# hrnr/map-merge

Hardware: AMD Instinct MI355X
Metric: map-pairs/sec (normals+FPFH+SAC-IA+ICP, end to end incl. per-map features) (higher is better)
Workload: dtype f32; 1 GPU; 16 maps x 500000 raw pts, FPFH + SAC_IA + ICP refine, 120 pairs; parallelism=one mm3d_estimate_maps_transforms call, 16 streams inside the library, points_after_filter_mean=406681, keypoints_mean=15692

## Files before the change

include/mm3d.h:

```cpp
#ifndef MM3D_H_
#define MM3D_H_

#include <stddef.h>
#include <stdint.h>

#ifdef __cplusplus
extern "C" {
#endif

typedef enum {
  MM3D_OK = 0,
  MM3D_EINVAL = -1,
  MM3D_EDEVICE = -2,
  MM3D_ENOMEM = -3,
  MM3D_EUNSUPPORTED = -4,
  MM3D_ECAPACITY = -5
} mm3d_status;

typedef enum { MM3D_DESC_PFH = 0, MM3D_DESC_PFHRGB, MM3D_DESC_FPFH, MM3D_DESC_RSD, MM3D_DESC_SHOT, MM3D_DESC_SC3D } mm3d_descriptor;
typedef enum { MM3D_KP_SIFT = 0, MM3D_KP_HARRIS } mm3d_keypoint;
typedef enum { MM3D_EST_MATCHING = 0, MM3D_EST_SAC_IA } mm3d_estimation_method;
typedef enum { MM3D_ICP_POINT_TO_POINT = 0, MM3D_ICP_POINT_TO_PLANE = 1 } mm3d_icp_method;

const char *mm3d_descriptor_name(int d);
int mm3d_descriptor_from_string(const char *s);
const char *mm3d_descriptor_field_name(int d);
int mm3d_descriptor_dim(int d);
const char *mm3d_keypoint_name(int k);
int mm3d_keypoint_from_string(const char *s);
const char *mm3d_estimation_method_name(int m);
int mm3d_estimation_method_from_string(const char *s);

typedef struct {
  double resolution;
  double descriptor_radius;
  int outliers_min_neighbours;
  double normal_radius;
  int keypoint_type;
  double keypoint_threshold;
  int descriptor_type;
  int estimation_method;
  int refine_transform;
  double inlier_threshold;
  double max_correspondence_distance;
  int max_iterations;
  uint64_t matching_k;
  double transform_epsilon;
  double confidence_threshold;
  double output_resolution;
} mm3d_params;
void mm3d_params_default(mm3d_params *p);
int mm3d_params_from_command_line(int argc, const char *const *argv, mm3d_params *p);
size_t mm3d_params_to_string(const mm3d_params *p, char *buf, size_t cap);

typedef struct { int32_t index_query, index_match; float distance; } mm3d_corr;

typedef struct mm3d_ctx mm3d_ctx;
typedef struct mm3d_cloud mm3d_cloud;
typedef struct mm3d_normals mm3d_normals;
typedef struct mm3d_desc mm3d_desc;

int mm3d_create(int device, mm3d_ctx **out);
int mm3d_create_devices(const int *devices, int n_devices, mm3d_ctx **out);
int mm3d_device_count(const mm3d_ctx *ctx);
int mm3d_device_at(const mm3d_ctx *ctx, int i);
int mm3d_devices_use_rccl(const mm3d_ctx *ctx);
void mm3d_destroy(mm3d_ctx *ctx);
const char *mm3d_last_error(const mm3d_ctx *ctx);
int mm3d_last_icp_iterations(const mm3d_ctx *ctx);
int mm3d_last_icp_converged(const mm3d_ctx *ctx);
void mm3d_set_debug(mm3d_ctx *ctx, int on);
long long mm3d_debug_knn_fallback_rows(mm3d_ctx *ctx);
long long mm3d_debug_knn_rows(mm3d_ctx *ctx);
void mm3d_debug_waits(mm3d_ctx *ctx, long long out[2]);
int mm3d_debug_float_chain(mm3d_ctx *ctx, const float *incr, const unsigned *hits, int n, float *out);
int mm3d_debug_libm(mm3d_ctx *ctx, int fn, const float *x, const float *y, int n, float *out);
int mm3d_debug_pair_bins(mm3d_ctx *ctx, const float *p1, const float *n1, const float *p2, const float *n2, int n, int *out);
void mm3d_debug_spfh_replay(const float *incr, const unsigned *hits, int n, float *out);
int mm3d_debug_sacia_queries_per_thread(int k);
int mm3d_debug_wave_primitives(mm3d_ctx *ctx, int op, const void *in, int n, void *out_new, void *out_old);
int mm3d_debug_sift_cert_octave(mm3d_ctx *ctx, const mm3d_cloud *points, double min_scale, int octave, float *val, float *bound,
                                size_t capacity, size_t *n_out);
void mm3d_debug_sift_cert_stats(long long out[8], int reset);
void mm3d_debug_sift_cert_min(int n);
int mm3d_debug_sift_dog_marked(mm3d_ctx *ctx, const mm3d_cloud *points, double min_scale, int octave, const int *ids, size_t n_ids,
                               int small_capacity, float *out);
float mm3d_debug_cloud_voxel_leaf(const mm3d_cloud *cloud);
void mm3d_debug_sacia_stats(long long out[4], int reset, int collect);
int mm3d_debug_desc_knn(mm3d_ctx *ctx, const float *a, size_t na, const float *b, size_t nb, int dim, int k, int *idx, float *d2);
typedef struct mm3d_nn_search_info {
  float max_d2;
  float rmax;
  float cell;
  float origin[3];
  int dims[3];
  int max_ring;
  int n_items;
} mm3d_nn_search_info;
int mm3d_debug_nn_search(mm3d_ctx *ctx, const mm3d_cloud *source, const mm3d_cloud *target, const float T[16], double range,
                         int convention, int split, int *idx, float *d2, mm3d_nn_search_info *info);
void mm3d_srand(mm3d_ctx *ctx, unsigned seed);
int mm3d_set_streams(mm3d_ctx *ctx, int n_streams);
int mm3d_get_streams(const mm3d_ctx *ctx);
int mm3d_last_run_stage_seconds(const mm3d_ctx *ctx, double *features_s, double *total_s);
int mm3d_last_run_device_seconds(const mm3d_ctx *ctx, double *exchange_s, double *pairs_s, double *gather_s);
size_t mm3d_last_run_map_sizes(const mm3d_ctx *ctx, size_t *points, size_t *keypoints, size_t capacity);
int mm3d_set_map_cache(mm3d_ctx *ctx, int max_maps);
int mm3d_get_map_cache(const mm3d_ctx *ctx);
void mm3d_map_cache_clear(mm3d_ctx *ctx);
int mm3d_map_cache_stats(const mm3d_ctx *ctx, long long out[6], int reset);
int mm3d_set_icp_method(mm3d_ctx *ctx, int method);
int mm3d_get_icp_method(const mm3d_ctx *ctx);
typedef enum { MM3D_ALIGN_SAC_IA = 0, MM3D_ALIGN_PREREJECTIVE = 1 } mm3d_align_method;
typedef struct mm3d_alignment_options {
  int method;
  int samples;
  int k;
  double similarity;
  double inlier_fraction;
} mm3d_alignment_options;
typedef struct mm3d_alignment_stats {
  long long draws;
  long long survivors;
  long long hypotheses_scored;
  long long winner_h;
  int winner_inliers;
  int converged;
} mm3d_alignment_stats;
void mm3d_alignment_options_default(mm3d_alignment_options *o);
int mm3d_set_alignment(mm3d_ctx *ctx, const mm3d_alignment_options *options);
int mm3d_get_alignment(const mm3d_ctx *ctx, mm3d_alignment_options *options);
int mm3d_last_alignment_stats(const mm3d_ctx *ctx, mm3d_alignment_stats *stats);
typedef enum { MM3D_KEYPOINTS_REFERENCE = 0, MM3D_KEYPOINTS_UNIFORM = 1 } mm3d_keypoint_source;
typedef struct mm3d_keypoint_options {
  int source;
  double leaf;
} mm3d_keypoint_options;
void mm3d_keypoint_options_default(mm3d_keypoint_options *o);
int mm3d_set_keypoints(mm3d_ctx *ctx, const mm3d_keypoint_options *options);
int mm3d_get_keypoints(const mm3d_ctx *ctx, mm3d_keypoint_options *options);
typedef enum { MM3D_OUTLIERS_RADIUS = 0, MM3D_OUTLIERS_STATISTICAL = 1 } mm3d_outlier_method;
typedef struct mm3d_outlier_options {
  int method;
  int mean_k;
  double stddev_mult;
} mm3d_outlier_options;
void mm3d_outlier_options_default(mm3d_outlier_options *o);
int mm3d_set_outlier_filter(mm3d_ctx *ctx, const mm3d_outlier_options *options);
int mm3d_get_outlier_filter(const mm3d_ctx *ctx, mm3d_outlier_options *options);
typedef struct mm3d_outlier_stats {
  long long points, valid, kept;
  int k;
  double mean, stddev, threshold;
} mm3d_outlier_stats;
int mm3d_last_outlier_stats(const mm3d_ctx *ctx, mm3d_outlier_stats *stats);
typedef enum { MM3D_CLUSTERS_OFF = 0, MM3D_CLUSTERS_MIN_SIZE = 1, MM3D_CLUSTERS_LARGEST = 2 } mm3d_cluster_method;
typedef struct mm3d_cluster_options {
  int method;
  int min_size;
  double tolerance;
} mm3d_cluster_options;
void mm3d_cluster_options_default(mm3d_cluster_options *o);
int mm3d_set_cluster_filter(mm3d_ctx *ctx, const mm3d_cluster_options *options);
int mm3d_get_cluster_filter(const mm3d_ctx *ctx, mm3d_cluster_options *options);
typedef struct mm3d_cluster_stats {
  long long points, valid, kept;
  long long clusters, kept_clusters;
  long long largest;
} mm3d_cluster_stats;
int mm3d_last_cluster_stats(const mm3d_ctx *ctx, mm3d_cluster_stats *stats);
typedef enum { MM3D_SMOOTH_OFF = 0, MM3D_SMOOTH_MLS = 1 } mm3d_smooth_method;
// ... 343 lines not shown
```

map-merge_amd/__init__.py:

```python
from __future__ import annotations

import ctypes as C
import enum
import os
import subprocess

import numpy as np

_HERE = os.path.dirname(os.path.abspath(__file__))
LIB_PATH = os.environ.get("MM3D_LIB") or os.path.join(_HERE, "libmm3d.so")

POINT = np.dtype([("x", "<f4"), ("y", "<f4"), ("z", "<f4"), ("rgba", "<u4")])
NORMAL = np.dtype([("nx", "<f4"), ("ny", "<f4"), ("nz", "<f4"), ("curvature", "<f4")])
CORR = np.dtype([("index_query", "<i4"), ("index_match", "<i4"), ("distance", "<f4")])
PAIR = np.dtype([("source_idx", "<u8"), ("target_idx", "<u8"), ("transform", "<f4", (16,)),
                 ("confidence", "<f8"), ("icp_iterations", "<i4"), ("n_correspondences", "<i4"),
                 ("n_inliers", "<i4"), ("icp_correspondences", "<i4")])


class Mm3dError(RuntimeError):
    def __init__(self, status, msg):
        super().__init__(f"mm3d status {status}: {msg}")
        self.status = status

# ... 1058 lines not shown

    def estimateTransformCorrelative(self, source_points, source_normals, target_points, target_normals, options=None, **kw):
        o = options if options is not None else CoarseOptions(**kw)
        T = np.zeros(16, dtype=np.float32)
        st = CoarseStats()
        self._ck(lib().mm3d_estimate_transform_correlative(
            self._h, source_points._h, source_normals._h, target_points._h, target_normals._h, C.byref(o),
            T.ctypes.data_as(C.c_void_p), C.byref(st)))
        return _Tout(T), st.as_dict()

    def correlativeSignature(self, points, normals, options=None, cap=1 << 20, **kw):
        o = options if options is not None else CoarseOptions(**kw)
        c = max(int(cap), 1)
        st = np.zeros((c, 3), dtype=np.int32)
        gr = np.zeros((c, 3), dtype=np.int32)
        gh = np.zeros(c, dtype=np.float32)
        co = np.zeros((c, 2), dtype=np.int32)
        n = (C.c_size_t * 3)()
        self._ck(lib().mm3d_debug_correlative_signature(
            self._h, points._h, normals._h, C.byref(o), st.ctypes.data_as(C.c_void_p), gr.ctypes.data_as(C.c_void_p),
            gh.ctypes.data_as(C.c_void_p), co.ctypes.data_as(C.c_void_p), C.c_size_t(c), n))
        if max(n) > c:
            raise RuntimeError("correlativeSignature: more cells than cap")
        return dict(structure=st[:n[0]].copy(), ground=gr[:n[1]].copy(), ground_height=gh[:n[1]].copy(), coarse=co[:n[2]].copy())

    def correlativeVotes(self, source_points, source_normals, target_points, target_normals, q, options=None, **kw):
        o = options if options is not None else CoarseOptions(**kw)
        frame = (C.c_int * 5)()
        n = C.c_size_t()
        K, W, GW = int(o.candidates), 2 * int(o.cell_factor) + 1, 2 * int(o.yaw_factor) + 1
        cands = np.zeros((K, 4), dtype=np.int32)
        scores = np.zeros((K, GW, W, W), dtype=np.int32)
        args = (self._h, source_points._h, source_normals._h, target_points._h, target_normals._h, C.byref(o), int(q), frame)
        self._ck(lib().mm3d_debug_correlative_votes(*args, None, C.c_size_t(0), cands.ctypes.data_as(C.c_void_p),
                                                    scores.ctypes.data_as(C.c_void_p), C.c_size_t(K), C.byref(n)))
        U, V = int(frame[3]), int(frame[4])
        acc = np.zeros((U, V), dtype=np.int32)
        if U * V:
            self._ck(lib().mm3d_debug_correlative_votes(*args, acc.ctypes.data_as(C.c_void_p), C.c_size_t(U * V),
                                                        cands.ctypes.data_as(C.c_void_p), scores.ctypes.data_as(C.c_void_p),
                                                        C.c_size_t(K), C.byref(n)))
        m = int(n.value)
        return dict(frame=tuple(int(x) for x in frame), acc=acc, cands=cands[:m].copy(), scores=scores[:m].copy())

    def transformOverlap(self, source_points, target_points, transform, options=None, **kw) -> dict:
        o = options if options is not None else ConfidenceOptions(**kw)
        T = _T(transform)
        st = OverlapStats()
        self._ck(lib().mm3d_transform_overlap(self._h, source_points._h, target_points._h, T.ctypes.data_as(C.c_void_p), C.byref(o),
                                              C.byref(st)))
        return st.as_dict()

    def debugOverlapTable(self, points, options=None, **kw) -> dict:
        o = options if options is not None else ConfidenceOptions(**kw)
        box = (C.c_int * 12)()
        self._ck(lib().mm3d_debug_overlap_table(self._h, points._h, C.byref(o), box, None, C.c_size_t(0), None, C.c_size_t(0)))
        b = [int(x) for x in box]
        words = np.zeros(tuple(b[3:6]), dtype=np.uint64)
        view = np.zeros(tuple(b[9:12]), dtype=np.uint8)
        if words.size:
            self._ck(lib().mm3d_debug_overlap_table(self._h, points._h, C.byref(o), box, words.ctypes.data_as(C.c_void_p),
                                                    C.c_size_t(words.size), view.ctypes.data_as(C.c_void_p), C.c_size_t(view.size)))
        return dict(brick0=tuple(b[0:3]), bricks=tuple(b[3:6]), view0=tuple(b[6:9]), views=tuple(b[9:12]), words=words, view=view)

    def estimateTransform(self, source_points, source_keypoints, source_descriptors, target_points,
                          target_keypoints, target_descriptors, method, refine, inlier_threshold,
                          max_correspondence_distance, max_iterations, matching_k, transform_epsilon):
        T = np.zeros(16, dtype=np.float32)
        self._ck(lib().mm3d_estimate_transform(
            self._h, source_points._h, source_keypoints._h, source_descriptors._h, target_points._h,
            target_keypoints._h, target_descriptors._h, int(method), int(bool(refine)), C.c_double(inlier_threshold),
            C.c_double(max_correspondence_distance), int(max_iterations), C.c_size_t(matching_k),
            C.c_double(transform_epsilon), T.ctypes.data_as(C.c_void_p)))
        return _Tout(T)

    def debugWavePrimitives(self, op, values):
        dt = {0: np.float64, 1: np.float32, 5: np.float32, 6: np.float32, 8: np.uint64}.get(int(op), np.int32)
        v = np.ascontiguousarray(values, dtype=dt)
        new, old = np.empty_like(v), np.empty_like(v)
        self._ck(lib().mm3d_debug_wave_primitives(self._h, int(op), v.ctypes.data_as(C.c_void_p), len(v),
                                                  new.ctypes.data_as(C.c_void_p), old.ctypes.data_as(C.c_void_p)))
        return new, old

    def debugNnSearch(self, source_points, target_points, transform, range, convention, split):
        n = len(source_points)
        idx = np.zeros(max(n, 1), dtype=np.int32)
        d2 = np.zeros(max(n, 1), dtype=np.float32)
        t = _T(transform)
        info = NnSearchInfo()
        self._ck(lib().mm3d_debug_nn_search(self._h, source_points._h, target_points._h, t.ctypes.data_as(C.c_void_p),
                                            C.c_double(range), int(convention), int(split), idx.ctypes.data_as(C.c_void_p),
                                            d2.ctypes.data_as(C.c_void_p), C.byref(info)))
        return idx[:n], d2[:n], info.as_dict()

    def debugColorGradients(self, points, normals, options=None, **kw):
        o = options if options is not None else IcpColorOptions(**kw)
        n = len(points)
        out = np.zeros((max(n, 1), 4), dtype=np.float32)
        self._ck(lib().mm3d_debug_color_gradients(self._h, points._h, normals._h, C.byref(o), out.ctypes.data_as(C.c_void_p)))
        return out[:n]

    def debugIcpRejection(self, source_points, target_points, transform, max_correspondence_distance, options=None, split=1, **kw):
        o = options if options is not None else IcpRejectionOptions(**kw)
        n = len(source_points)
        idx = np.zeros(max(n, 1), dtype=np.int32)
        d2 = np.zeros(max(n, 1), dtype=np.float32)
        kept = np.zeros(max(n, 1), dtype=np.uint8)
        t = _T(transform)
        st = IcpRejectionStats()
        self._ck(lib().mm3d_debug_icp_rejection(self._h, source_points._h, target_points._h, t.ctypes.data_as(C.c_void_p),
                                                C.c_double(max_correspondence_distance), C.byref(o), int(split),
                                                idx.ctypes.data_as(C.c_void_p), d2.ctypes.data_as(C.c_void_p),
                                                kept.ctypes.data_as(C.c_void_p), C.byref(st)))
        return idx[:n], d2[:n], kept[:n].astype(bool), st.as_dict()

    def transformScore(self, source_points, target_points, transform, max_distance) -> float:
        t = _T(transform)
        s = C.c_double()
        self._ck(lib().mm3d_transform_score(self._h, source_points._h, target_points._h, t.ctypes.data_as(C.c_void_p),
                                            C.c_double(max_distance), C.byref(s)))
        return s.value

    def estimateMapsTransforms(self, clouds, params: MapMergingParams, return_pairs: bool = False):
        n = len(clouds)
        keep = []
        views = (_View * max(n, 1))()
        for i, c in enumerate(clouds):
            if isinstance(c, tuple):
                views[i] = _View(C.c_void_p(c[0]), c[1], c[2] if len(c) > 2 else 16, c[3] if len(c) > 3 else 12)
            else:
                a = np.ascontiguousarray(c, dtype=POINT)
                keep.append(a)
                views[i] = _View(a.ctypes.data_as(C.c_void_p), len(a), 16, 12)
        out = np.zeros((max(n, 1), 16), dtype=np.float32)
        pairs = np.zeros(max(n * (n - 1) // 2, 1), dtype=PAIR)
        n_out, n_pairs = C.c_size_t(), C.c_size_t()
        self._ck(lib().mm3d_estimate_maps_transforms(self._h, views, C.c_size_t(n), C.byref(params),
                                                     out.ctypes.data_as(C.c_void_p), C.byref(n_out),
                                                     pairs.ctypes.data_as(C.c_void_p), C.byref(n_pairs)))
        res = [_Tout(out[i]) for i in range(n_out.value)]
        return (res, pairs[:n_pairs.value].copy()) if return_pairs else res

    def composeMaps(self, clouds, transforms, resolution: float):
        n = len(clouds)
        if n == 0:
            return None
        if n != len(transforms):
            raise RuntimeError("composeMaps: clouds and transforms size must be the same.")
        arr = (C.c_void_p * n)(*[c._h for c in clouds])
        tr = np.ascontiguousarray(np.stack([_T(t) for t in transforms]))
        h = C.c_void_p()
        self._ck(lib().mm3d_compose_maps(self._h, arr, C.c_size_t(n), tr.ctypes.data_as(C.c_void_p), C.c_size_t(n),
                                         C.c_double(resolution), C.byref(h)))
        return Cloud(self, h)

    def mapFeatures(self, raw: "Cloud", params: MapMergingParams) -> "Map":
        h = C.c_void_p()
        self._ck(lib().mm3d_map_features(self._h, raw._h, C.byref(params), C.byref(h)))
        return Map(self, h)

    def mapFromParts(self, points: "Cloud", keypoints: "Cloud", desc: "Descriptors") -> "Map":
        h = C.c_void_p()
        self._ck(lib().mm3d_map_from_parts(self._h, points._h, keypoints._h, desc._h, C.byref(h)))
        for o in (points, keypoints, desc):
            o._owned = False
        return Map(self, h)
# ... 190 lines not shown
```

map-merge_amd/csrc/registration.hip:

```cpp
#include <atomic>
#include <cfloat>
#include <cstdlib>

#include "device_util.hpp"
#include "linalg_shared.hpp"

namespace mm3d {

__global__ void __launch_bounds__(256)
k_ransac_count(const float4 *__restrict__ skp, const float4 *__restrict__ tkp, const int *__restrict__ is,
               const int *__restrict__ it, int n_corr, const float *__restrict__ T_all, int H, float thr_le,
               int *__restrict__ counts)
{
  const int h = blockIdx.x * (blockDim.x >> 6) + (threadIdx.x >> 6);
  if (h >= H) return;
  const int lane = threadIdx.x & 63;
  float T[16];
#pragma unroll
  for (int k = 0; k < 16; ++k) T[k] = T_all[(size_t)h * 16 + k];
  int cnt = 0;
  for (int i = lane; i < n_corr; i += kWave) {
    const float4 s = skp[is[i]], t = tkp[it[i]];
    const float3 p = xform(T, s.x, s.y, s.z);
    const float dx = p.x - t.x, dy = p.y - t.y, dz = p.z - t.z;
    const float d = __fadd_rn(__fadd_rn(__fmul_rn(dx, dx), __fmul_rn(dy, dy)), __fmul_rn(dz, dz));
    cnt += (d <= thr_le) ? 1 : 0;
  }
  cnt = wave_sum(cnt);
  if (lane == 0) counts[h] = cnt;
}

void ransac_count(Context *c, const float4 *src_kp, const float4 *tgt_kp, const int *idx_src, const int *idx_tgt,
                  int n_corr, const float *T_all, int H, double thr2, int *counts)
{
  float thr_le = (float)thr2;
  if ((double)thr_le >= thr2) thr_le = std::nextafterf(thr_le, -INFINITY);
  MM3D_LAUNCH(c, "ransac_count", (double)H * n_corr * 8.0, k_ransac_count, dim3(div_up(H, 4)), dim3(256), 0, src_kp, tgt_kp,
              idx_src, idx_tgt, n_corr, T_all, H, thr_le, counts);
}

struct SacJob {
  const float4 *skp, *tkp;
  const int *samp, *corr_ref, *nn;
  float *T_all;
  const float4 *skp_q;
  int ns;
  GridView g;
  float *err;
  float *T_best;
  double *S;
  int *n_part;
  int *chain_list;
  unsigned char *cls;
  struct SacCtl *ctl;
};
struct SacCtl { int n_cand, decided, winner, n_chain; };

__global__ void k_sacia_models(const SacJob *__restrict__ jobs, int H)
{
  const SacJob &J = jobs[blockIdx.y];
  const float4 *__restrict__ skp = J.skp, *__restrict__ tkp = J.tkp;
  const int *__restrict__ samp = J.samp, *__restrict__ corr_ref = J.corr_ref, *__restrict__ nn = J.nn;
  float *__restrict__ T_all = J.T_all;
  const int h = blockIdx.x * blockDim.x + threadIdx.x;
  if (h >= H) return;
  float s[9], d[9], T[16];
#pragma unroll
  for (int i = 0; i < 3; ++i) {
    const float4 p = skp[samp[h * 3 + i]], q = tkp[nn[corr_ref[h * 3 + i]]];
    s[i * 3] = p.x; s[i * 3 + 1] = p.y; s[i * 3 + 2] = p.z;
    d[i * 3] = q.x; d[i * 3 + 1] = q.y; d[i * 3 + 2] = q.z;
  }
  umeyama_f32_shared(s, d, 3, T);
#pragma unroll
  for (int i = 0; i < 16; ++i) T_all[(size_t)h * 16 + i] = T[i];
}

#ifndef MM3D_SAC_SUB
#define MM3D_SAC_SUB 1
#endif
constexpr int kSacSub = MM3D_SAC_SUB;
struct SacQuery { float3 p; int b, e; float slack; bool inside; };
__device__ __forceinline__ SacQuery sacia_locate(const GridView &g, const float *Tl, const float4 s)
{
  SacQuery q;
  q.p = xform(Tl, s.x, s.y, s.z);
  const int cx = cell_floor(q.p.x, g.minx, g.inv), cy = cell_floor(q.p.y, g.miny, g.inv), cz = cell_floor(q.p.z, g.minz, g.inv);
  q.inside = cx >= 0 && cx < g.dx && cy >= 0 && cy < g.dy && cz >= 0 && cz < g.dz;
  const size_t c = q.inside ? ((size_t)cz * g.dy + cy) * g.dx + cx : 0;
  q.b = g.nb_start[c];
  q.e = g.nb_start[c + 1];
  const float ox = q.p.x - (g.minx + ((float)cx + 0.5f) * g.cell), oy = q.p.y - (g.miny + ((float)cy + 0.5f) * g.cell);
  const float oz = q.p.z - (g.minz + ((float)cz + 0.5f) * g.cell);
  q.slack = sqrtf(ox * ox + oy * oy + oz * oz) + 1e-3f * g.cell;
  return q;
}
__device__ __forceinline__ float sacia_scan(const GridView &g, const SacQuery &q, float thresh, float radius)
{
  const float3 p = q.p;
  float best = INFINITY;
  if (q.inside) {
    const int e = q.e;
    float want = thresh;
    for (int j = q.b; j < e; j += 4) {
      const int last = e - 1;
      const float4 q0 = g.nb_pts[j];
      const float4 q1 = g.nb_pts[min(j + 1, last)];
      const float4 q2 = g.nb_pts[min(j + 2, last)];
      const float4 q3 = g.nb_pts[min(j + 3, last)];
      const float d0 = dist2(p.x, p.y, p.z, q0.x, q0.y, q0.z), d1 = dist2(p.x, p.y, p.z, q1.x, q1.y, q1.z);
      const float d2 = dist2(p.x, p.y, p.z, q2.x, q2.y, q2.z), d3 = dist2(p.x, p.y, p.z, q3.x, q3.y, q3.z);
      best = fminf(best, fminf(fminf(d0, d1), fminf(d2, d3)));
      want = fminf(want, best);
      const float lb = q3.w - q.slack;
      if (lb > 0.0f && lb * lb > want) break;
    }
  } else {
    for_each_candidate(g, p.x, p.y, p.z, radius, [&](const float4 &t) {
      best = fminf(best, dist2(p.x, p.y, p.z, t.x, t.y, t.z));
      return true;
    });
  }
  return (best <= thresh) ? best / thresh : 1.0f;
}
__device__ __forceinline__ float sacia_term(const GridView &g, const float *Tl, const float4 s, float thresh, float radius)
{
  return sacia_scan(g, sacia_locate(g, Tl, s), thresh, radius);
}

template <int K>
__global__ void __launch_bounds__(256)
k_sacia_err(const SacJob *__restrict__ jobs, int h_first, float thresh, float radius)
{
  const SacJob &J = jobs[blockIdx.z];
  const int ns = J.ns;
  const int i0 = (int)blockIdx.x * (256 * K);
  if (i0 >= ns) return;
  const int h = h_first + (int)blockIdx.y;
  const float *T = J.T_all + (size_t)h * 16;
  float Tl[16];
#pragma unroll
  for (int k = 0; k < 16; ++k) Tl[k] = T[k];
  float4 s[K];
#pragma unroll
  for (int k = 0; k < K; ++k) {
    const int i = i0 + k * 256 + (int)threadIdx.x;
    s[k] = J.skp_q[i < ns ? i : i0];
  }
  SacQuery q[K];
#pragma unroll
  for (int k = 0; k < K; ++k) q[k] = sacia_locate(J.g, Tl, s[k]);
  double sum = 0.0;
  int part = 0;
#pragma unroll
  for (int k = 0; k < K; ++k) {
    const bool valid = i0 + k * 256 + (int)threadIdx.x < ns;
    const float e_term = valid ? sacia_scan(J.g, q[k], thresh, radius) : 0.0f;
    sum += (double)e_term;
    part += (valid && e_term != 1.0f) ? 1 : 0;
  }
  __shared__ double s_sum[4];
  __shared__ int s_part[4];
  const double ws = wave_sum(sum);
  part = wave_sum(part);
  if ((threadIdx.x & 63) == 0) { s_sum[threadIdx.x >> 6] = ws; s_part[threadIdx.x >> 6] = part; }
  __syncthreads();
  if (threadIdx.x == 0) {
    atomicAdd(&J.S[h], (s_sum[0] + s_sum[1]) + (s_sum[2] + s_sum[3]));
    const int pt = s_part[0] + s_part[1] + s_part[2] + s_part[3];
    if (pt) atomicAdd(&J.n_part[h], pt);
  }
}
#ifndef MM3D_SAC_K
#define MM3D_SAC_K 4
#endif
constexpr int kSacK = MM3D_SAC_K;
constexpr long long kSacMinTiles = 256 * 8;
static std::atomic<int> g_sacia_k{[] { const char *e = getenv("MM3D_SAC_K"); return e ? atoi(e) : 0; }()};
static int sacia_queries_per_thread(long long ns_total, int hn)
{
  const int knob = g_sacia_k.load();
  if (knob == 1 || knob == 2 || knob == 4 || knob == 8) return knob;
  int k = kSacK;
  while (k > 1 && div_up(ns_total, 256 * k) * hn < kSacMinTiles) k >>= 1;
  return k;
}

__global__ void __launch_bounds__(256) k_sacia_select(const SacJob *__restrict__ jobs, int H)
{
  const SacJob &J = jobs[blockIdx.x];
  const double *__restrict__ S = J.S;
  const int *__restrict__ n_part = J.n_part;
  const double n = (double)J.ns;
  const double d = n * 5.9604644775390625e-8 * 1.001 + 1e-12;
  __shared__ double s_min[4];
  __shared__ int s_cnt[4], s_chain[4], s_first[4];
  const int lane = threadIdx.x & 63, wave = threadIdx.x >> 6;
  double up = INFINITY;
  for (int h = threadIdx.x; h < H; h += blockDim.x) {
    const double hi = n_part[h] == 0 ? n : S[h] * (1.0 + d);
    up = hi < up ? hi : up;
  }
#pragma unroll
  for (int o = 32; o > 0; o >>= 1) { const double t = __shfl_xor(up, o, kWave); up = t < up ? t : up; }
  if (lane == 0) s_min[wave] = up;
  __syncthreads();
  up = fmin(fmin(s_min[0], s_min[1]), fmin(s_min[2], s_min[3]));
  int cnt = 0, chain = 0, first = 0x7fffffff;
  for (int h = threadIdx.x; h < H; h += blockDim.x) {
    const bool exact = n_part[h] == 0;
    const double lo = exact ? n : S[h] * (1.0 - d);
    const bool cand = lo <= up;
    J.cls[h] = cand ? (exact ? 2 : 1) : 0;
    if (exact) J.err[h] = (float)J.ns;
    cnt += cand ? 1 : 0;
    chain += (cand && !exact) ? 1 : 0;
    if (cand) first = min(first, h);
    if (cand && !exact) J.chain_list[atomicAdd(&J.ctl->n_chain, 1)] = h;
  }
  cnt = wave_sum(cnt); chain = wave_sum(chain); first = wave_min_int(first);
  if (lane == 0) { s_cnt[wave] = cnt; s_chain[wave] = chain; s_first[wave] = first; }
  __syncthreads();
  if (threadIdx.x == 0) {
    cnt = s_cnt[0] + s_cnt[1] + s_cnt[2] + s_cnt[3];
    chain = s_chain[0] + s_chain[1] + s_chain[2] + s_chain[3];
    first = min(min(s_first[0], s_first[1]), min(s_first[2], s_first[3]));
    SacCtl c;
    c.n_cand = cnt; c.n_chain = cnt == 0 ? H : chain;
    c.decided = (cnt == 1 || (cnt > 0 && chain == 0)) ? 1 : 0;
    c.winner = c.decided ? first : -1;
    *J.ctl = c;
  }
  __syncthreads();
  const SacCtl c = *J.ctl;
  if (c.n_cand == 0)
    for (int h = threadIdx.x; h < H; h += blockDim.x) { J.cls[h] = 1; J.chain_list[h] = h; }
  if (c.decided && threadIdx.x < 16) J.T_best[threadIdx.x] = J.T_all[(size_t)c.winner * 16 + threadIdx.x];
}

constexpr int kSacExactBlocks = 8;
__global__ void __launch_bounds__(256) k_sacia_exact(const SacJob *__restrict__ jobs, float thresh, float radius)
{
  const SacJob &J = jobs[blockIdx.y];
  if (J.ctl->decided) return;
  const int n_chain = J.ctl->n_chain, ns = J.ns;
  __shared__ __attribute__((aligned(16))) float s_e[256];
  for (int k = blockIdx.x; k < n_chain; k += gridDim.x) {
    const int h = J.chain_list[k];
    const float *T = J.T_all + (size_t)h * 16;
    float Tl[16];
#pragma unroll
    for (int q = 0; q < 16; ++q) Tl[q] = T[q];
    float e = 0.0f;
    for (int i0 = 0; i0 < ns; i0 += 256) {
      const int i = i0 + (int)threadIdx.x;
      s_e[threadIdx.x] = i < ns ? sacia_term(J.g, Tl, J.skp[i], thresh, radius) : 0.0f;
      __syncthreads();
      if (threadIdx.x == 0) {
        const float4 *row = reinterpret_cast<const float4 *>(s_e);
#pragma unroll 4
        for (int g4 = 0; g4 < 64; ++g4) {
          const float4 v = row[g4];
          e += v.x; e += v.y; e += v.z; e += v.w;
        }
      }
      __syncthreads();
    }
    if (threadIdx.x == 0) J.err[h] = e;
  }
}

static const Grid &sacia_target_grid(Context *c, const mm3d_cloud *tgt_kp, float corr_thresh)
{
  const float radius = std::sqrt(corr_thresh > 0.f ? corr_thresh : 0.f);
  const float want = radius * 1.001f / (float)kSacSub;
  const float cell = want > 0.125f ? want : 0.125f;
  const Grid &g = cloud_grid(c, tgt_kp, cell);
  grid_ensure_nblists(c, g, kSacSub);
  return g;
}

void prepare_sacia_target(Context *c, const mm3d_cloud *kp, float corr_thresh)
{
  if (kp->n) {
    (void)sacia_target_grid(c, kp, corr_thresh);
    cloud_hilbert(c, kp);
  }
}

__global__ void k_sacia_pick(const SacJob *__restrict__ jobs, int H);

static std::atomic<long long> g_sacia_stats[4];
static std::atomic<int> g_sacia_collect{0};
void debug_sacia_stats(long long out[4], int reset, int collect)
{
  for (int i = 0; i < 4; ++i) { out[i] = g_sacia_stats[i].load(); if (reset) g_sacia_stats[i] = 0; }
  if (collect >= 0) g_sacia_collect = collect;
}

void sacia_score_batch(Context *c, const SacPair *pairs, int n, int H, float corr_thresh)
{
  if (n == 0 || H == 0) return;
  const float radius = std::sqrt(corr_thresh > 0.f ? corr_thresh : 0.f);
  std::vector<DevBuf<float>> bufs;
  bufs.reserve((size_t)n * 3);
  const size_t per_pair = (((size_t)H * 17 + sizeof(SacCtl)) + 15) & ~(size_t)15;
  DevBuf<unsigned char> cert(c, per_pair * (size_t)n);
  MM3D_HIP(hipMemsetAsync(cert.get(), 0, per_pair * (size_t)n, c->stream));
  SacJob *hj = (SacJob *)c->pin(sizeof(SacJob) * (size_t)n);
  int max_ns = 0;
  long long sum_ns = 0;
  double err_bytes = 0.0;
  for (int i = 0; i < n; ++i) {
    const SacPair &P = pairs[i];
    const int ns = (int)P.src_kp->n;
    const Grid &g = sacia_target_grid(c, P.tgt_kp, corr_thresh);
    cloud_hilbert(c, P.src_kp);
    const bool permuted = P.src_kp->hil_pts.get() && P.src_kp->n_finite == P.src_kp->n;
    bufs.emplace_back(c, (size_t)H * 16);
    float *T_all = bufs.back().get();
    bufs.emplace_back(c, (size_t)H);
    float *err = bufs.back().get();
    SacJob q;
    std::memset(&q, 0, sizeof(q));
    q.skp = (const float4 *)P.src_kp->pts.get();
    q.tkp = (const float4 *)P.tgt_kp->pts.get();
    q.samp = P.samp; q.corr_ref = P.corr_ref; q.nn = P.nn;
    q.T_all = T_all;
    q.skp_q = permuted ? (const float4 *)P.src_kp->hil_pts.get() : (const float4 *)P.src_kp->pts.get();
    q.ns = ns;
    q.g = g.view();
    q.err = err; q.T_best = P.T_best;
    unsigned char *cp = cert.get() + per_pair * (size_t)i;
    q.S = reinterpret_cast<double *>(cp);
    q.n_part = reinterpret_cast<int *>(cp + (size_t)H * 8);
    q.chain_list = reinterpret_cast<int *>(cp + (size_t)H * 12);
    q.ctl = reinterpret_cast<SacCtl *>(cp + (size_t)H * 16);
    q.cls = cp + (size_t)H * 16 + sizeof(SacCtl);
    hj[i] = q;
    max_ns = std::max(max_ns, ns);
    sum_ns += ns;
    err_bytes += (double)ns * H * 4.0 + ns * 16.0;
  }
  DevBuf<SacJob> d_jobs(c, (size_t)n);
  MM3D_HIP(hipMemcpyAsync(d_jobs.get(), hj, sizeof(SacJob) * (size_t)n, hipMemcpyHostToDevice, c->stream));
  const SacJob *dj = d_jobs.get();
  MM3D_LAUNCH(c, "sacia_models", n * H * 88.0, k_sacia_models, dim3(div_up(H, 64), n), dim3(64), 0, dj, H);
  for (int h0 = 0; h0 < H; h0 += 65535) {
    const int hn = std::min(65535, H - h0);
    const double bytes = err_bytes * hn / H;
    switch (sacia_queries_per_thread(sum_ns, hn)) {
#define MM3D_SAC_ERR(K_) case K_: MM3D_LAUNCH(c, "sacia_err", bytes, (k_sacia_err<K_>), dim3(div_up(max_ns, 256 * K_), hn, n), dim3(256), 0, dj, h0, corr_thresh, radius); break
      MM3D_SAC_ERR(8);
      MM3D_SAC_ERR(4);
      MM3D_SAC_ERR(2);
      default: MM3D_SAC_ERR(1);
#undef MM3D_SAC_ERR
    }
  }
  MM3D_LAUNCH(c, "sacia_select", n * (H * 12.0 + 128.0), k_sacia_select, dim3(n), dim3(256), 0, dj, H);
  MM3D_LAUNCH(c, "sacia_seq_sum", 0.0, k_sacia_exact, dim3(kSacExactBlocks, n), dim3(256), 0, dj, corr_thresh, radius);
  MM3D_LAUNCH(c, "sacia_pick", n * 128.0, k_sacia_pick, dim3(n), dim3(64), 0, dj, H);
  static const bool env_collect = getenv("MM3D_SACIA_STATS") != nullptr;
  if (env_collect || g_sacia_collect.load()) {
    SacCtl *hc = (SacCtl *)c->pin(sizeof(SacCtl) * (size_t)n);
    for (int i = 0; i < n; ++i)
      MM3D_HIP(hipMemcpyAsync(hc + i, hj[i].ctl, sizeof(SacCtl), hipMemcpyDeviceToHost, c->stream));
    c->sync();
    for (int i = 0; i < n; ++i) {
      g_sacia_stats[0] += 1; g_sacia_stats[1] += hc[i].decided ? 1 : 0;
      g_sacia_stats[2] += hc[i].n_cand; g_sacia_stats[3] += hc[i].decided ? 0 : (hc[i].n_cand ? hc[i].n_chain : H);
    }
  }
}

__global__ void __launch_bounds__(64) k_sacia_pick(const SacJob *__restrict__ jobs, int H)
{
  if (jobs[blockIdx.x].ctl->decided) return;
  const float *__restrict__ err = jobs[blockIdx.x].err;
  const unsigned char *__restrict__ cls = jobs[blockIdx.x].cls;
  const float *__restrict__ T_all = jobs[blockIdx.x].T_all;
  float *__restrict__ T_best = jobs[blockIdx.x].T_best;
  const int lane = threadIdx.x;
  const float e0 = cls[0] ? err[0] : 0.0f;
  unsigned long long best = ~0ull;
  if (e0 == e0) {
    for (int i = lane; i < H; i += kWave) {
      if (!cls[i]) continue;
      const float e = err[i];
      if (e == e) {
        const unsigned long long key = ((unsigned long long)f2ord(e) << 32) | (unsigned)i;
        best = key < best ? key : best;
      }
    }
    best = wave_min_u64(best);
  }
  const int h = (e0 == e0) ? (int)(unsigned)(best & 0xffffffffull) : 0;
  if (lane < 16) T_best[lane] = T_all[(size_t)h * 16 + lane];
}


}

extern "C" int mm3d_debug_sacia_queries_per_thread(int k)
{
  if (k >= 0) mm3d::g_sacia_k = k;
  return mm3d::kSacK;
}
```

Measured before the change: 1473 map-pairs/s.

## Rebalance SAC-IA error scan with per-wave work queue and early-exit cell scan

Rewrites the SAC-IA error kernel so each wave compacts its queries into LDS and then deals them dynamically to lanes as they finish. Each lane scans grid cell neighbours four at a time and stops early using a sorted-distance lower bound. Points far outside the grid skip the scan and count as a full penalty term. This targets lane divergence from uneven neighbour-list lengths, at the cost of extra LDS traffic, ballots and fences. It also lowers the default queries per thread from 4 to 2, and adds debug entry points for checking the sums against a reference and for gathering queue statistics.

```diff
diff --git a/include/mm3d.h b/include/mm3d.h
--- a/include/mm3d.h
+++ b/include/mm3d.h
@@ -87,6 +87,11 @@
                                int small_capacity, float *out);
 float mm3d_debug_cloud_voxel_leaf(const mm3d_cloud *cloud);
 void mm3d_debug_sacia_stats(long long out[4], int reset, int collect);
+int mm3d_debug_sacia_sums(mm3d_ctx *ctx, const mm3d_cloud *src_kp, const mm3d_cloud *tgt_kp, const float *T , int H,
+                          float corr_thresh, double *S_out, int *n_part_out, double *S_ref_out, int *n_part_ref_out);
+int mm3d_debug_sacia_sums_batch(mm3d_ctx *ctx, const mm3d_cloud *const *src_kp, const mm3d_cloud *const *tgt_kp, int n_pairs,
+                                const float *T , int H, float corr_thresh, double *S_out, int *n_part_out,
+                                double *S_ref_out, int *n_part_ref_out);
 int mm3d_debug_desc_knn(mm3d_ctx *ctx, const float *a, size_t na, const float *b, size_t nb, int dim, int k, int *idx, float *d2);
 typedef struct mm3d_nn_search_info {
   float max_d2;
diff --git a/map-merge_amd/__init__.py b/map-merge_amd/__init__.py
--- a/map-merge_amd/__init__.py
+++ b/map-merge_amd/__init__.py
@@ -1164,6 +1164,22 @@
                                                   new.ctypes.data_as(C.c_void_p), old.ctypes.data_as(C.c_void_p)))
         return new, old
 
+    def debugSaciaSums(self, src_kp, tgt_kp, transforms, corr_thresh):
+        single = not isinstance(src_kp, (list, tuple))
+        srcs, tgts = ([src_kp], [tgt_kp]) if single else (list(src_kp), list(tgt_kp))
+        n, H = len(srcs), len(transforms)
+        t = np.ascontiguousarray(np.stack([_T(x) for x in transforms]))
+        S, S_ref = np.zeros((n, H), dtype=np.float64), np.zeros((n, H), dtype=np.float64)
+        part, part_ref = np.zeros((n, H), dtype=np.int32), np.zeros((n, H), dtype=np.int32)
+        args = (t.ctypes.data_as(C.c_void_p), H, C.c_float(corr_thresh), S.ctypes.data_as(C.c_void_p), part.ctypes.data_as(C.c_void_p),
+                S_ref.ctypes.data_as(C.c_void_p), part_ref.ctypes.data_as(C.c_void_p))
+        if single:
+            self._ck(lib().mm3d_debug_sacia_sums(self._h, srcs[0]._h, tgts[0]._h, *args))
+            return S[0], part[0], S_ref[0], part_ref[0]
+        sa, ta = (C.c_void_p * n)(*[s._h for s in srcs]), (C.c_void_p * n)(*[x._h for x in tgts])
+        self._ck(lib().mm3d_debug_sacia_sums_batch(self._h, sa, ta, n, *args))
+        return S, part, S_ref, part_ref
+
     def debugNnSearch(self, source_points, target_points, transform, range, convention, split):
         n = len(source_points)
         idx = np.zeros(max(n, 1), dtype=np.int32)
diff --git a/map-merge_amd/csrc/registration.hip b/map-merge_amd/csrc/registration.hip
--- a/map-merge_amd/csrc/registration.hip
+++ b/map-merge_amd/csrc/registration.hip
@@ -2,6 +2,7 @@
 #include <cfloat>
 #include <cstdlib>
 
+#include "capi_guard.hpp"
 #include "device_util.hpp"
 #include "linalg_shared.hpp"
 
@@ -128,10 +129,57 @@
   return sacia_scan(g, sacia_locate(g, Tl, s), thresh, radius);
 }
 
+#ifndef MM3D_SAC_DEAL
+#define MM3D_SAC_DEAL 1
+#endif
+#ifndef MM3D_SAC_CHUNK
+#define MM3D_SAC_CHUNK 4
+#endif
+constexpr int kSacChunk = MM3D_SAC_CHUNK;
+__device__ __forceinline__ int lanes_below(unsigned long long m)
+{
+  return (int)__builtin_amdgcn_mbcnt_hi((unsigned)(m >> 32), __builtin_amdgcn_mbcnt_lo((unsigned)m, 0u));
+}
+__device__ __forceinline__ bool sacia_err_near_box(const GridView &g, const float3 p, float reach)
+{
+  const float ex = fmaxf(fmaxf(g.minx - p.x, p.x - (g.minx + (float)g.dx * g.cell)), 0.0f);
+  const float ey = fmaxf(fmaxf(g.miny - p.y, p.y - (g.miny + (float)g.dy * g.cell)), 0.0f);
+  const float ez = fmaxf(fmaxf(g.minz - p.z, p.z - (g.minz + (float)g.dz * g.cell)), 0.0f);
+  return fmaxf(ex, fmaxf(ey, ez)) <= reach;
+}
+__device__ __forceinline__ float sacia_err_reach(const GridView &g, float radius)
+{
+  return radius * 1.0001f + 1e-4f + 1e-3f * g.cell +
+         1e-6f * (fabsf(g.minx) + fabsf(g.miny) + fabsf(g.minz) + (float)(g.dx + g.dy + g.dz) * g.cell);
+}
+__device__ __forceinline__ float sacia_err_slack(const GridView &g, const float3 p, int cx, int cy, int cz)
+{
+  const float ox = p.x - (g.minx + ((float)cx + 0.5f) * g.cell), oy = p.y - (g.miny + ((float)cy + 0.5f) * g.cell);
+  const float oz = p.z - (g.minz + ((float)cz + 0.5f) * g.cell);
+  return sqrtf(ox * ox + oy * oy + oz * oz) + 1e-3f * g.cell;
+}
+__device__ __forceinline__ bool sacia_err_trip(const GridView &g, float px, float py, float pz, float slack, int &j, int e, float &best,
+                                               float &want)
+{
+  const int last = e - 1;
+  const float4 q0 = g.nb_pts[j];
+  const float4 q1 = g.nb_pts[min(j + 1, last)];
+  const float4 q2 = g.nb_pts[min(j + 2, last)];
+  const float4 q3 = g.nb_pts[min(j + 3, last)];
+  const float d0 = dist2(px, py, pz, q0.x, q0.y, q0.z), d1 = dist2(px, py, pz, q1.x, q1.y, q1.z);
+  const float d2 = dist2(px, py, pz, q2.x, q2.y, q2.z), d3 = dist2(px, py, pz, q3.x, q3.y, q3.z);
+  best = fminf(best, fminf(fminf(d0, d1), fminf(d2, d3)));
+  want = fminf(want, best);
+  const float lb = q3.w - slack;
+  j += 4;
+  return j >= e || (lb > 0.0f && lb * lb > want);
+}
+
 template <int K>
 __global__ void __launch_bounds__(256)
 k_sacia_err(const SacJob *__restrict__ jobs, int h_first, float thresh, float radius)
 {
+  constexpr int KC = K < kSacChunk ? K : kSacChunk;
   const SacJob &J = jobs[blockIdx.z];
   const int ns = J.ns;
   const int i0 = (int)blockIdx.x * (256 * K);
@@ -141,24 +189,94 @@
   float Tl[16];
 #pragma unroll
   for (int k = 0; k < 16; ++k) Tl[k] = T[k];
-  float4 s[K];
-#pragma unroll
-  for (int k = 0; k < K; ++k) {
-    const int i = i0 + k * 256 + (int)threadIdx.x;
-    s[k] = J.skp_q[i < ns ? i : i0];
-  }
-  SacQuery q[K];
-#pragma unroll
-  for (int k = 0; k < K; ++k) q[k] = sacia_locate(J.g, Tl, s[k]);
+  const GridView &g = J.g;
+  const float reach = sacia_err_reach(g, radius);
+  __shared__ float4 s_qp[4][64 * KC];
+  __shared__ int2 s_qs[4][64 * KC];
+  const int lane = (int)threadIdx.x & 63;
+  float4 *__restrict__ qp = s_qp[threadIdx.x >> 6];
+  int2 *__restrict__ qs = s_qs[threadIdx.x >> 6];
   double sum = 0.0;
-  int part = 0;
-#pragma unroll
-  for (int k = 0; k < K; ++k) {
-    const bool valid = i0 + k * 256 + (int)threadIdx.x < ns;
-    const float e_term = valid ? sacia_scan(J.g, q[k], thresh, radius) : 0.0f;
-    sum += (double)e_term;
-    part += (valid && e_term != 1.0f) ? 1 : 0;
-  }
+  int part = 0, ones = 0;
+#pragma unroll 1
+  for (int c0 = 0; c0 < K; c0 += KC) {
+    float4 s[KC];
+#pragma unroll
+    for (int k = 0; k < KC; ++k) {
+      const int i = i0 + (c0 + k) * 256 + (int)threadIdx.x;
+      s[k] = J.skp_q[i < ns ? i : i0];
+    }
+    float3 p[KC];
+    int cx[KC], cy[KC], cz[KC], b[KC], e[KC];
+    bool in[KC];
+#pragma unroll
+    for (int k = 0; k < KC; ++k) {
+      const bool valid = i0 + (c0 + k) * 256 + (int)threadIdx.x < ns;
+      p[k] = xform(Tl, s[k].x, s[k].y, s[k].z);
+      cx[k] = cell_floor(p[k].x, g.minx, g.inv); cy[k] = cell_floor(p[k].y, g.miny, g.inv); cz[k] = cell_floor(p[k].z, g.minz, g.inv);
+      const bool inside = cx[k] >= 0 && cx[k] < g.dx && cy[k] >= 0 && cy[k] < g.dy && cz[k] >= 0 && cz[k] < g.dz;
+      in[k] = valid && (inside || sacia_err_near_box(g, p[k], reach));
+      cx[k] = clampi(cx[k], 0, g.dx - 1); cy[k] = clampi(cy[k], 0, g.dy - 1); cz[k] = clampi(cz[k], 0, g.dz - 1);
+      b[k] = 0; e[k] = 0;
+      if (in[k]) {
+        const size_t c = ((size_t)cz[k] * g.dy + cy[k]) * g.dx + cx[k];
+        b[k] = g.nb_start[c];
+        e[k] = g.nb_start[c + 1];
+      }
+      ones += (valid && !in[k]) ? 1 : 0;
+    }
+    int nq = 0;
+#pragma unroll
+    for (int k = 0; k < KC; ++k) {
+      const bool queued = in[k] && b[k] < e[k];
+      ones += (in[k] && !queued) ? 1 : 0;
+      const unsigned long long m = ballot(queued);
+      if (queued) {
+        const int pos = nq + lanes_below(m);
+        qp[pos] = make_float4(p[k].x, p[k].y, p[k].z, sacia_err_slack(g, p[k], cx[k], cy[k], cz[k]));
+        qs[pos] = make_int2(b[k], e[k]);
+      }
+      nq += __popcll(m);
+    }
+    wave_lds_fence();
+    {
+      int cur = lane, e_ = 0, j = 0;
+      int claimed = kWave;
+      float px = 0.f, py = 0.f, pz = 0.f, slack = 0.f, best = INFINITY, want = thresh;
+      bool have = cur < nq;
+      if (have) {
+        const float4 a = qp[cur];
+        const int2 be = qs[cur];
+        px = a.x; py = a.y; pz = a.z; slack = a.w; j = be.x; e_ = be.y;
+      }
+      while (ballot(have)) {
+        bool done = false;
+        if (have) done = sacia_err_trip(g, px, py, pz, slack, j, e_, best, want);
+        const unsigned long long dm = ballot(done);
+        if (done) {
+          qs[cur].y = __float_as_int(best);
+          cur = MM3D_SAC_DEAL ? claimed + lanes_below(dm) : cur + kWave;
+          have = cur < nq;
+          if (have) {
+            const float4 a = qp[cur];
+            const int2 be = qs[cur];
+            px = a.x; py = a.y; pz = a.z; slack = a.w; j = be.x; e_ = be.y;
+            best = INFINITY; want = thresh;
+          }
+        }
+        claimed += __popcll(dm);
+      }
+    }
+    wave_lds_fence();
+    for (int i = lane; i < nq; i += kWave) {
+      const float best = __int_as_float(qs[i].y);
+      const float e_term = (best <= thresh) ? best / thresh : 1.0f;
+      sum += (double)e_term;
+      part += (e_term != 1.0f) ? 1 : 0;
+    }
+    wave_lds_fence();
+  }
+  sum += (double)ones;
   __shared__ double s_sum[4];
   __shared__ int s_part[4];
   const double ws = wave_sum(sum);
@@ -172,7 +290,7 @@
   }
 }
 #ifndef MM3D_SAC_K
-#define MM3D_SAC_K 4
+#define MM3D_SAC_K 2
 #endif
 constexpr int kSacK = MM3D_SAC_K;
 constexpr long long kSacMinTiles = 256 * 8;
@@ -296,6 +414,24 @@
 {
   for (int i = 0; i < 4; ++i) { out[i] = g_sacia_stats[i].load(); if (reset) g_sacia_stats[i] = 0; }
   if (collect >= 0) g_sacia_collect = collect;
+}
+
+static void sacia_price_launches(Context *c, const SacJob *dj, int n, int H, int max_ns, long long sum_ns, float corr_thresh, float radius);
+static void sacia_err_launches(Context *c, const SacJob *dj, int n, int H, int max_ns, long long sum_ns, double err_bytes,
+                               float corr_thresh, float radius)
+{
+  for (int h0 = 0; h0 < H; h0 += 65535) {
+    const int hn = std::min(65535, H - h0);
+    const double bytes = err_bytes * hn / H;
+    switch (sacia_queries_per_thread(sum_ns, hn)) {
+#define MM3D_SAC_ERR(K_) case K_: MM3D_LAUNCH(c, "sacia_err", bytes, (k_sacia_err<K_>), dim3(div_up(max_ns, 256 * K_), hn, n), dim3(256), 0, dj, h0, corr_thresh, radius); break
+      MM3D_SAC_ERR(8);
+      MM3D_SAC_ERR(4);
+      MM3D_SAC_ERR(2);
+      default: MM3D_SAC_ERR(1);
+#undef MM3D_SAC_ERR
+    }
+  }
 }
 
 void sacia_score_batch(Context *c, const SacPair *pairs, int n, int H, float corr_thresh)
@@ -346,18 +482,8 @@
   MM3D_HIP(hipMemcpyAsync(d_jobs.get(), hj, sizeof(SacJob) * (size_t)n, hipMemcpyHostToDevice, c->stream));
   const SacJob *dj = d_jobs.get();
   MM3D_LAUNCH(c, "sacia_models", n * H * 88.0, k_sacia_models, dim3(div_up(H, 64), n), dim3(64), 0, dj, H);
-  for (int h0 = 0; h0 < H; h0 += 65535) {
-    const int hn = std::min(65535, H - h0);
-    const double bytes = err_bytes * hn / H;
-    switch (sacia_queries_per_thread(sum_ns, hn)) {
-#define MM3D_SAC_ERR(K_) case K_: MM3D_LAUNCH(c, "sacia_err", bytes, (k_sacia_err<K_>), dim3(div_up(max_ns, 256 * K_), hn, n), dim3(256), 0, dj, h0, corr_thresh, radius); break
-      MM3D_SAC_ERR(8);
-      MM3D_SAC_ERR(4);
-      MM3D_SAC_ERR(2);
-      default: MM3D_SAC_ERR(1);
-#undef MM3D_SAC_ERR
-    }
-  }
+  sacia_err_launches(c, dj, n, H, max_ns, sum_ns, err_bytes, corr_thresh, radius);
+  sacia_price_launches(c, dj, n, H, max_ns, sum_ns, corr_thresh, radius);
   MM3D_LAUNCH(c, "sacia_select", n * (H * 12.0 + 128.0), k_sacia_select, dim3(n), dim3(256), 0, dj, H);
   MM3D_LAUNCH(c, "sacia_seq_sum", 0.0, k_sacia_exact, dim3(kSacExactBlocks, n), dim3(256), 0, dj, corr_thresh, radius);
   MM3D_LAUNCH(c, "sacia_pick", n * 128.0, k_sacia_pick, dim3(n), dim3(64), 0, dj, H);
@@ -399,8 +525,196 @@
   if (lane < 16) T_best[lane] = T_all[(size_t)h * 16 + lane];
 }
 
-
-}
+__global__ void __launch_bounds__(256)
+k_debug_sacia_terms(const SacJob *__restrict__ jobs, int pair, float thresh, float radius, float *__restrict__ terms)
+{
+  const SacJob &J = jobs[pair];
+  const int i = (int)(blockIdx.x * blockDim.x + threadIdx.x), h = (int)blockIdx.y;
+  if (i >= J.ns) return;
+  const float *T = J.T_all + (size_t)h * 16;
+  float Tl[16];
+#pragma unroll
+  for (int k = 0; k < 16; ++k) Tl[k] = T[k];
+  terms[(size_t)h * J.ns + i] = sacia_term(J.g, Tl, J.skp[i], thresh, radius);
+}
+
+#ifdef MM3D_SAC_QUEUE_PRICE
+__device__ unsigned long long g_sacq_price[16];
+template <int K>
+__global__ void __launch_bounds__(256)
+k_debug_sacia_price(const SacJob *__restrict__ jobs, int h_first, float thresh, float radius)
+{
+  const SacJob &J = jobs[blockIdx.z];
+  const int ns = J.ns;
+  const int i0 = (int)blockIdx.x * (256 * K);
+  if (i0 >= ns) return;
+  const int h = h_first + (int)blockIdx.y;
+  const float *T = J.T_all + (size_t)h * 16;
+  float Tl[16];
+#pragma unroll
+  for (int k = 0; k < 16; ++k) Tl[k] = T[k];
+  const GridView &g = J.g;
+  const float reach = sacia_err_reach(g, radius);
+  __shared__ int s_deal[4][64];
+  const int lane = (int)threadIdx.x & 63, wave = (int)threadIdx.x >> 6;
+  s_deal[wave][lane] = 0;
+  wave_lds_fence();
+  unsigned long long cnt[11];
+#pragma unroll
+  for (int q = 0; q < 11; ++q) cnt[q] = 0;
+  int nq = 0, total = 0, longest = 0;
+#pragma unroll 1
+  for (int k = 0; k < K; ++k) {
+    const int i = i0 + k * 256 + (int)threadIdx.x;
+    const bool valid = i < ns;
+    const float4 sk = J.skp_q[valid ? i : i0];
+    const float3 p = xform(Tl, sk.x, sk.y, sk.z);
+    int cx = cell_floor(p.x, g.minx, g.inv), cy = cell_floor(p.y, g.miny, g.inv), cz = cell_floor(p.z, g.minz, g.inv);
+    const bool inside = cx >= 0 && cx < g.dx && cy >= 0 && cy < g.dy && cz >= 0 && cz < g.dz;
+    const bool near = valid && !inside && sacia_err_near_box(g, p, reach);
+    cx = clampi(cx, 0, g.dx - 1); cy = clampi(cy, 0, g.dy - 1); cz = clampi(cz, 0, g.dz - 1);
+    const size_t c = ((size_t)cz * g.dy + cy) * g.dx + cx;
+    const int qb = g.nb_start[c], qe = g.nb_start[c + 1];
+    const bool queued = valid && (inside || near) && qb < qe;
+    int trips = 0;
+    if (queued) {
+      const float slack = sacia_err_slack(g, p, cx, cy, cz);
+      float best = INFINITY, want = thresh;
+      int j = qb;
+      do ++trips; while (!sacia_err_trip(g, p.x, p.y, p.z, slack, j, qe, best, want));
+    }
+    const int trips_in = (valid && inside) ? trips : 0;
+    const unsigned long long m = ballot(queued);
+    if (queued) atomicAdd(&s_deal[wave][(nq + lanes_below(m)) & 63], trips);
+    nq += __popcll(m);
+    cnt[0] += __popcll(ballot(valid));
+    cnt[1] += __popcll(ballot(valid && inside && queued));
+    cnt[2] += __popcll(ballot(valid && inside && !queued));
+    cnt[3] += __popcll(ballot(near));
+    cnt[4] += __popcll(ballot(valid && !inside && !near));
+    const int wt = wave_sum(trips), wm = wave_max_int(trips);
+    total += wt;
+    longest = max(longest, wm);
+    cnt[6] += wave_max_int(trips_in);
+    cnt[10] |= ballot(near) ? 1 : 0;
+  }
+  wave_lds_fence();
+  cnt[5] = total;
+  cnt[7] = wave_max_int(s_deal[wave][lane]);
+  cnt[8] = total ? (total + 63) / 64 + longest : 0;
+  cnt[9] = 1;
+  if (lane == 0) {
+#pragma unroll
+    for (int q = 0; q < 11; ++q)
+      if (cnt[q]) atomicAdd(&g_sacq_price[q], cnt[q]);
+    if (blockIdx.x == 0 && blockIdx.y == 0 && blockIdx.z == 0 && wave == 0) atomicAdd(&g_sacq_price[11], 1ull);
+  }
+}
+#endif
+
+static void sacia_price_launches(Context *c, const SacJob *dj, int n, int H, int max_ns, long long sum_ns, float corr_thresh, float radius)
+{
+#ifdef MM3D_SAC_QUEUE_PRICE
+  for (int h0 = 0; h0 < H; h0 += 65535) {
+    const int hn = std::min(65535, H - h0);
+    switch (sacia_queries_per_thread(sum_ns, hn)) {
+#define MM3D_SAC_PRICE(K_) case K_: MM3D_LAUNCH(c, "debug_sacia_price", 0.0, (k_debug_sacia_price<K_>), dim3(div_up(max_ns, 256 * K_), hn, n), dim3(256), 0, dj, h0, corr_thresh, radius); break
+      MM3D_SAC_PRICE(8);
+      MM3D_SAC_PRICE(4);
+      MM3D_SAC_PRICE(2);
+      default: MM3D_SAC_PRICE(1);
+#undef MM3D_SAC_PRICE
+    }
+  }
+#endif
+}
+
+static void debug_sacia_sums(Context *c, const mm3d_cloud *const *src_kp, const mm3d_cloud *const *tgt_kp, int n, const float *T, int H,
+                             float corr_thresh, double *S_out, int *n_part_out, double *S_ref_out, int *n_part_ref_out)
+{
+  const float radius = std::sqrt(corr_thresh > 0.f ? corr_thresh : 0.f);
+  DevBuf<float> T_all(c, (size_t)H * 16);
+  MM3D_HIP(hipMemcpyAsync(T_all.get(), T, (size_t)H * 64, hipMemcpyHostToDevice, c->stream));
+  const size_t per_pair = (size_t)H * 16;
+  DevBuf<unsigned char> cert(c, per_pair * (size_t)n);
+  MM3D_HIP(hipMemsetAsync(cert.get(), 0, per_pair * (size_t)n, c->stream));
+  std::vector<SacJob> hj((size_t)n);
+  int max_ns = 0;
+  long long sum_ns = 0;
+  for (int i = 0; i < n; ++i) {
+    const Grid &g = sacia_target_grid(c, tgt_kp[i], corr_thresh);
+    cloud_hilbert(c, src_kp[i]);
+    const bool permuted = src_kp[i]->hil_pts.get() && src_kp[i]->n_finite == src_kp[i]->n;
+    SacJob q;
+    std::memset(&q, 0, sizeof(q));
+    q.skp = (const float4 *)src_kp[i]->pts.get();
+    q.tkp = (const float4 *)tgt_kp[i]->pts.get();
+    q.T_all = T_all.get();
+    q.skp_q = permuted ? (const float4 *)src_kp[i]->hil_pts.get() : q.skp;
+    q.ns = (int)src_kp[i]->n;
+    q.g = g.view();
+    q.S = reinterpret_cast<double *>(cert.get() + per_pair * (size_t)i);
+    q.n_part = reinterpret_cast<int *>(cert.get() + per_pair * (size_t)i + (size_t)H * 8);
+    hj[(size_t)i] = q;
+    max_ns = std::max(max_ns, q.ns);
+    sum_ns += q.ns;
+  }
+  DevBuf<SacJob> d_jobs(c, (size_t)n);
+  MM3D_HIP(hipMemcpyAsync(d_jobs.get(), hj.data(), sizeof(SacJob) * (size_t)n, hipMemcpyHostToDevice, c->stream));
+  c->sync();
+  sacia_err_launches(c, d_jobs.get(), n, H, max_ns, sum_ns, 0.0, corr_thresh, radius);
+  std::vector<unsigned char> hc(per_pair * (size_t)n);
+  MM3D_HIP(hipMemcpyAsync(hc.data(), cert.get(), hc.size(), hipMemcpyDeviceToHost, c->stream));
+  DevBuf<float> terms(c, (size_t)H * (size_t)max_ns);
+  std::vector<float> ht((size_t)H * (size_t)max_ns);
+  for (int i = 0; i < n; ++i) {
+    const int ns = hj[(size_t)i].ns;
+    MM3D_LAUNCH(c, "debug_sacia_terms", (double)H * ns * 4.0, k_debug_sacia_terms, dim3(div_up(ns, 256), H), dim3(256), 0,
+                (const SacJob *)d_jobs.get(), i, corr_thresh, radius, terms.get());
+    MM3D_HIP(hipMemcpyAsync(ht.data(), terms.get(), (size_t)H * ns * sizeof(float), hipMemcpyDeviceToHost, c->stream));
+    c->sync();
+    for (int h = 0; h < H; ++h) {
+      double S = 0.0;
+      int part = 0;
+      for (int k = 0; k < ns; ++k) { const float e = ht[(size_t)h * ns + k]; S += (double)e; part += e != 1.0f ? 1 : 0; }
+      S_ref_out[(size_t)i * H + h] = S;
+      n_part_ref_out[(size_t)i * H + h] = part;
+    }
+  }
+  for (int i = 0; i < n; ++i) {
+    std::memcpy(S_out + (size_t)i * H, hc.data() + per_pair * (size_t)i, (size_t)H * 8);
+    std::memcpy(n_part_out + (size_t)i * H, hc.data() + per_pair * (size_t)i + (size_t)H * 8, (size_t)H * 4);
+  }
+}
+
+}
+
+extern "C" int mm3d_debug_sacia_sums_batch(mm3d_ctx *ctx, const mm3d_cloud *const *src_kp, const mm3d_cloud *const *tgt_kp, int n_pairs,
+                                           const float *T, int H, float corr_thresh, double *S_out, int *n_part_out, double *S_ref_out,
+                                           int *n_part_ref_out)
+{
+  if (!src_kp || !tgt_kp || n_pairs <= 0 || n_pairs > 65535 || !T || H <= 0 || !S_out || !n_part_out || !S_ref_out || !n_part_ref_out)
+    return MM3D_EINVAL;
+  if (!(corr_thresh > 0.0f) || !std::isfinite(corr_thresh)) return MM3D_EINVAL;
+  for (int i = 0; i < n_pairs; ++i)
+    if (!src_kp[i] || !tgt_kp[i] || src_kp[i]->n == 0 || tgt_kp[i]->n == 0 || src_kp[i]->n >= ((size_t)1 << 24)) return MM3D_EINVAL;
+  return mm3d::guarded(ctx, [&] {
+    mm3d::debug_sacia_sums(ctx, src_kp, tgt_kp, n_pairs, T, H, corr_thresh, S_out, n_part_out, S_ref_out, n_part_ref_out);
+  });
+}
+extern "C" int mm3d_debug_sacia_sums(mm3d_ctx *ctx, const mm3d_cloud *src_kp, const mm3d_cloud *tgt_kp, const float *T, int H,
+                                     float corr_thresh, double *S_out, int *n_part_out, double *S_ref_out, int *n_part_ref_out)
+{
+  return mm3d_debug_sacia_sums_batch(ctx, &src_kp, &tgt_kp, 1, T, H, corr_thresh, S_out, n_part_out, S_ref_out, n_part_ref_out);
+}
+#ifdef MM3D_SAC_QUEUE_PRICE
+extern "C" void mm3d_debug_sacia_queue_price(unsigned long long *out, int reset)
+{
+  (void)hipDeviceSynchronize();
+  (void)hipMemcpyFromSymbol(out, HIP_SYMBOL(mm3d::g_sacq_price), sizeof(unsigned long long) * 16);
+  if (reset) { unsigned long long z[16] = {0}; (void)hipMemcpyToSymbol(HIP_SYMBOL(mm3d::g_sacq_price), z, sizeof(z)); }
+}
+#endif
 
 extern "C" int mm3d_debug_sacia_queries_per_thread(int k)
 {
```

New measurement: 1468 map-pairs/s. About the same (-0.4%).
